# phlash/java-sdr

Hardware: NVIDIA B200
Metric: Msamples/s (complex IQ) through mix+FIR+FFT (higher is better)
Workload: dtype f32 (FFT/PSD) + f64 (tuner/decimator, reference order, bit-exact)

## Files before the change

include/jsdrcuda.h:

```cpp
#ifndef JSDRCUDA_H
#define JSDRCUDA_H

#include <stddef.h>
#include <stdint.h>

#ifdef __cplusplus
extern "C" {
#endif

#define JSDR_ABI_VERSION 2

typedef enum jsdr_status {
    JSDR_OK = 0,
    JSDR_EINVAL = -1,
    JSDR_ECUDA = -2,
    JSDR_ENOMEM = -3,
    JSDR_EUNSUPPORTED = -4,
    JSDR_ESTATE = -5,
    JSDR_EINTERNAL = -6
} jsdr_status;

enum { JSDR_MEM_HOST = 0, JSDR_MEM_DEVICE = 1 };

typedef struct jsdr_ctx jsdr_ctx;
// ... 82 lines not shown
                        int32_t *pixels, int mem);

int jsdr_fir_design(int f1, int f2, float rate, double w[21]);
int jsdr_fir_nco_table(int freq, float rate, int32_t *sig );
int jsdr_fir_create(jsdr_ctx *ctx, int nchan, int max_block_samples, jsdr_fir **out);
int jsdr_fir_destroy(jsdr_fir *f);
int jsdr_fir_set_weights(jsdr_fir *f, int chan, const double w[21]);
int jsdr_fir_filter_i32(jsdr_fir *f, const int32_t *in, int nsamples, int64_t chan_stride,
                        int32_t *out , int mem);
int jsdr_fir_complex_mod_i32(jsdr_ctx *ctx, const int32_t *a, const int32_t *b, int32_t *out,
                             int64_t npairs, int mem);

int jsdr_probe_table(int which, int32_t *out, int n);
int jsdr_probe_taps(double ds27[27], double dm65[65]);
int jsdr_probe_scout_thresholds(double inc, double *th1, double *th2);

int jsdr_pump_receive_s16(jsdr_fft *f, jsdr_bpsk *b, const int16_t *raw, int nblocks,
                          int ic, int qc, float *psd, int32_t *peak_bin, int mem);
int jsdr_pump_waterfall_s16(jsdr_fft *f, jsdr_bpsk *b, const int16_t *raw, int nblocks,
                            int ic, int qc, int width, uint32_t peak_rgb, int32_t *pixels,
                            float *peak, int32_t *peak_bin, int mem);

#ifdef __cplusplus
}
#endif
#endif
```

java-sdr_b200/csrc/bpsk.cu:

```cuda
#include <math.h>

#include <algorithm>
#include <cmath>
#include <stdlib.h>
#include <string.h>

#include <vector>

#include "fft_generic.cuh"
#include "handles.h"

namespace jsdr {
namespace bpsk {

constexpr double kTwoPi = 2.0 * 3.141592653589793;
constexpr double kInvTwoPi = 1.0 / kTwoPi;
constexpr int kTileOut = 128;
constexpr int kTileThreads = 128;
constexpr int kPrefetch = 21;
constexpr double kIdxScaleHi = 40.74366543152521;
constexpr double kIdxScaleLo = -9.306125250357089e-16;
constexpr int kDmTile = 128;

enum { FMT_F32 = 0, FMT_S16 = 1 };
// ... 163 lines not shown
            ph = p[k];
            const double ic = par[ch].inc;
            for (int w = 0; w < nfull; w++) {
                ckpt[(size_t)w * nchan + ch] = ph;
#pragma unroll 4
                for (int j = 0; j < 32; j++) ph = phase_step(ph, ic);
            }
        }
        if (S & 31) {
            const double ic = par[ch].inc;
            ckpt[(size_t)nfull * nchan + ch] = ph;
            for (int j = 0; j < (S & 31); j++) ph = phase_step(ph, ic);
        }
        phase_out[ch] = ph;
    }
}

__global__ void k_vco_scout(const double *__restrict__ state, double *__restrict__ state_out,
                            uint8_t *__restrict__ vco_ix, uint8_t *__restrict__ bit_roll, int NO, double vco_inc,
                            double bit_inc, double bit_time)
{
    if (threadIdx.x == 0) {
        double p = state[0];
        for (int m = 0; m < NO; m++) {
            p = phase_step(p, vco_inc);
            double q = __ddiv_rn(__dmul_rn(p, 256.0), kTwoPi);
            vco_ix[m] = (uint8_t)(__double2int_rz(q) & 255);
        }
        state_out[0] = p;
    } else if (threadIdx.x == 32) {
// ... 582 lines not shown
        return from_bits(lo);
    };
    th1 = last_false(wraps1);
    th2 = last_false(wraps2);
}

static ScoutChan scout_chan(double inc)
{
    ScoutChan c;
    c.inc = inc;
    c.th1 = c.th2 = c.pad = 0.0;
    if (inc > 0.0 && inc < 3.1) scout_thresholds(inc, c.th1, c.th2);
    return c;
}

int launch_scout(jsdr_bpsk *b, jsdr_bpsk::TunerPlan &P, int S)
{
    jsdr_ctx *ctx = b->ctx;
    ProfScope prof(ctx, JSDR_K_SCOUT, ctx->side);
    const int st = scout_threads(b), cpt = scout_cpt(b);
    static int scout_smem = 0;
    if (!scout_smem) scout_smem = env_int("JSDR_SCOUT_SMEM_KB", 1, 200, kScoutSmem / 1024) * 1024;
    static PerDeviceFlag attr_done;
    JSDR_TRY(attr_done.once(ctx->device, [&]() -> int {
        JSDR_CUDA(cudaFuncSetAttribute(k_tuner_scout<1>, cudaFuncAttributeMaxDynamicSharedMemorySize, scout_smem));
        JSDR_CUDA(cudaFuncSetAttribute(k_tuner_scout<2>, cudaFuncAttributeMaxDynamicSharedMemorySize, scout_smem));
        JSDR_CUDA(cudaFuncSetAttribute(k_tuner_scout<3>, cudaFuncAttributeMaxDynamicSharedMemorySize, scout_smem));
        JSDR_CUDA(cudaFuncSetAttribute(k_tuner_scout<4>, cudaFuncAttributeMaxDynamicSharedMemorySize, scout_smem));
        return JSDR_OK;
    }));
    const int per_cta = st * cpt;
    const int grid = (b->nchan + per_cta - 1) / per_cta;
    void (*kern)(const ScoutChan *, const double *, double *, double *, int, int) =
        cpt == 1 ? k_tuner_scout<1> : cpt == 2 ? k_tuner_scout<2> : cpt == 3 ? k_tuner_scout<3> : k_tuner_scout<4>;
// ... 112 lines not shown
    sp.in = mp.in;
    sp.chan_stride = mp.chan_stride;
    sp.S = S;
    sp.ic = mp.ic;
    sp.qc = mp.qc;
    sp.tu_dx56 = b->d_tu_dx56;
    sp.tu_inc = mp.tu_inc;
    sp.ckpt = mp.ckpt;
    sp.nchan = mp.nchan;
    sp.nchunks = (S + 31) / 32;
    sp.hist_in = mp.hist_in;
    sp.cossin = mp.cossin;
    sp.n0 = mp.n0;
    sp.NO = mp.NO;
    sp.ncw = (mp.nchan + 31) / 32;
    const int scout_ctas = (mp.nchan + scout_threads(b) - 1) / scout_threads(b);
    sp.grid = b->in_pump ? b->ctx->sm_count : std::max(b->ctx->sm_count - scout_ctas, b->ctx->sm_count / 2);
    sp.warps_per_cta = (FMT == FMT_S16) ? stream::kWarps : stream::kWarpsF32;
    const int resident = sp.grid * sp.warps_per_cta;
    static int segs_per_warp = 0;
    if (!segs_per_warp) segs_per_warp = env_int("JSDR_STREAM_SEGS", 1, 64, 10);
    int nseg = std::max(1, segs_per_warp * resident / sp.ncw);
    int R = (mp.NO + nseg - 1) / nseg;
    if (R < 64) R = 64;
    sp.R = R;
    sp.nseg = (mp.NO + R - 1) / R;
    sp.ds_out = mp.ds_out;
    sp.max_ds = mp.max_ds;
    sp.work_counter = reinterpret_cast<unsigned *>(b->d_nbits + b->nchan);
    for (int k = 0; k < stream::kMaxTaps; k++) {
        sp.taps[k] = (k < b->ntaps) ? b->h_taps[k] : 0.0;
        sp.tapsf[k] = (float)sp.taps[k];
// ... 82 lines not shown
        JSDR_CUDA(cudaMemsetAsync(b->d_nbits, 0, sizeof(int32_t) * b->nchan, ctx->aux));
        if (b->fec && b->stages >= 3 && b->d_bits) JSDR_TRY(jsdr_fec_after_bits(b));
        return JSDR_OK;
    }
    const int D = b->D;
    const int NO = (b->ds_cnt + S) / D;
    const int n0 = D - 1 - b->ds_cnt;
    const int nchan = b->nchan;

    jsdr_bpsk::TunerPlan &P = b->plan[b->plan_cur];
    const bool autotune = b->dofft != 0;
    if (autotune) JSDR_REQUIRE(S == b->max_block, JSDR_EINVAL, "auto-tune needs whole blocks of max_block_samples");
    JSDR_CUDA(cudaEventRecord(ctx->ev_fork, ctx->stream));
    JSDR_CUDA(cudaStreamWaitEvent(ctx->side, ctx->ev_fork, 0));
    JSDR_CUDA(cudaStreamWaitEvent(ctx->side2, ctx->ev_fork, 0));
    if (!autotune && !(P.valid && P.S == S)) JSDR_TRY(launch_scout(b, P, S));
    const int kb = b->bit_cur;
    if (b->stages >= 2 && NO > 0) {
        if (!(b->vco_ahead_valid && b->vco_ahead_NO == NO && b->vco_ahead_kb == kb)) JSDR_TRY(launch_vco_scout(b, NO, kb));
        b->vco_ahead_valid = false;
    }
    JSDR_CUDA(cudaEventRecord(ctx->ev_join, ctx->side));

    const void *d_in = in;
    if (mem == JSDR_MEM_HOST) {
        const size_t esz = (FMT == FMT_S16) ? 4 : 8;
        const size_t total = (chan_stride == 0) ? (size_t)S : (size_t)chan_stride * (nchan - 1) + S;
        if (b->in_cap < total * esz) {
            cudaFree(b->d_in);
            b->d_in = nullptr;
            b->in_cap = 0;
// ... 63 lines not shown
        kern<<<grid, kTileThreads, smem, ctx->stream>>>(mp);
        JSDR_TRY(launched(ctx, "k_mixdecim"));
    }
    if (b->ntaps > 1) {
        k_tuner_tail<FMT><<<nchan, 128, 0, ctx->stream>>>(mp);
        JSDR_TRY(launched(ctx, "k_tuner_tail"));
    }
    JSDR_CUDA(cudaEventRecord(P.consumed, ctx->stream));
    P.used = true;
    P.valid = false;
    b->d_tu_phase = P.phase_end;
    b->plan_cur ^= 1;
    {
        jsdr_bpsk::TunerPlan &Pn = b->plan[b->plan_cur];
        if (Pn.used) JSDR_CUDA(cudaStreamWaitEvent(ctx->side, Pn.consumed, 0));
        JSDR_TRY(launch_scout(b, Pn, S));
    }
    }
    b->ds_hist_cur ^= 1;
    b->ds_cnt = (b->ds_cnt + S) % D;
    b->cnt_raw += S;
    b->last_nds = NO;

    if (b->stages >= 2 && NO > 0) {
        JSDR_CUDA(cudaStreamWaitEvent(ctx->stream, b->ev_vco_ready, 0));
        b->vco_state_cur ^= 1;
        DmParams dp;
        dp.ds = b->d_ds_out;
        dp.max_ds = b->max_ds;
        dp.NO = NO;
        dp.vco_ix = b->d_vco_ix[kb];
// ... 96 lines not shown
            cudaGetLastError();                                      \
            return JSDR_ENOMEM;                                      \
        }                                                            \
        cudaMemsetAsync((ptr), 0, (bytes), ctx->stream);             \
    } while (0)
    ALLOC(b->d_taps, sizeof(double) * kMaxDsTaps);
    ALLOC(b->d_dmtaps, sizeof(double) * kDmTaps);
    ALLOC(b->d_cossin, sizeof(double) * 512);
    ALLOC(b->d_cossin2, sizeof(double2) * 257);
    ALLOC(b->d_tu_inc, sizeof(double) * nc);
    ALLOC(b->d_tu_par, sizeof(ScoutChan) * nc);
    ALLOC(b->d_tu_dx, sizeof(unsigned long long) * nc);
    ALLOC(b->d_tu_dx56, sizeof(unsigned long long) * nc);
    ALLOC(b->d_tu_phase0, sizeof(double) * nc);
    b->d_tu_phase = b->d_tu_phase0;
    for (int i = 0; i < 2; i++) {
        ALLOC(b->plan[i].ckpt, sizeof(double) * nc * b->max_words);
        ALLOC(b->plan[i].phase_end, sizeof(double) * nc);
        cudaEventCreateWithFlags(&b->plan[i].ready, cudaEventDisableTiming);
        cudaEventCreateWithFlags(&b->plan[i].consumed, cudaEventDisableTiming);
    }
    ALLOC(b->d_ds_hist[0], sizeof(double2) * kMaxDsTaps * nc);
    ALLOC(b->d_ds_hist[1], sizeof(double2) * kMaxDsTaps * nc);
    ALLOC(b->d_ds_out, sizeof(double2) * nc * b->max_ds);
    ALLOC(b->d_vco_state, sizeof(double) * 4);
    ALLOC(b->d_ts, sizeof(TimingState) * nc);
    ALLOC(b->d_nbits, sizeof(int32_t) * (nc + 1));
#undef ALLOC
    std::vector<double> cossin(512);
    for (int n = 0; n < 256; n++) {
// ... 16 lines not shown
        cs2[2 * n + 1] = cossin[256 + n];
    }
    cs2[512] = cs2[513] = 1.0;
    for (int i = 0; i < kMaxDsTaps; i++) b->h_taps[i] = taps[i];
    std::vector<TimingState> ts(nchan);
    memset(ts.data(), 0, sizeof(TimingState) * nc);
    for (int c = 0; c < nchan; c++) ts[c].dmEnergyOut = 1.0;
    int rc = upload(ctx, b->d_cossin, cossin.data(), sizeof(double) * 512);
    if (rc == JSDR_OK) rc = upload(ctx, b->d_taps, taps.data(), sizeof(double) * kMaxDsTaps);
    if (rc == JSDR_OK) rc = upload(ctx, b->d_dmtaps, dmt.data(), sizeof(double) * kDmTaps);
    if (rc == JSDR_OK) rc = upload(ctx, b->d_tu_inc, inc.data(), sizeof(double) * nc);
    if (rc == JSDR_OK) {
        std::vector<ScoutChan> par(nchan);
        for (int c = 0; c < nchan; c++) par[c] = scout_chan(inc[c]);
        rc = upload(ctx, b->d_tu_par, par.data(), sizeof(ScoutChan) * nc);
    }
    if (rc == JSDR_OK) rc = upload(ctx, b->d_tu_dx, dx.data(), sizeof(unsigned long long) * nc);
    if (rc == JSDR_OK) rc = upload(ctx, b->d_tu_dx56, dx56.data(), sizeof(unsigned long long) * nc);
    if (rc == JSDR_OK) rc = upload(ctx, b->d_cossin2, cs2.data(), sizeof(double) * 2 * 257);
    if (rc == JSDR_OK) rc = upload(ctx, b->d_ts, ts.data(), sizeof(TimingState) * nc);
    if (rc != JSDR_OK) {
        jsdr_bpsk_destroy(b);
        return rc;
    }
    *out = b;
    return JSDR_OK;
} JSDR_CATCH_ALL

extern "C" int jsdr_bpsk_destroy(jsdr_bpsk *b)
try {
    if (!b) return JSDR_OK;
    b->ctx->bind();
    cudaStreamSynchronize(b->ctx->side);
    cudaStreamSynchronize(b->ctx->side2);
    cudaStreamSynchronize(b->ctx->stream);
    cudaStreamSynchronize(b->ctx->aux);
    if (b->ds_read_pending) cudaStreamSynchronize(b->ctx->copy_out);
    if (b->ev_dm_ready) cudaEventDestroy(b->ev_dm_ready);
    if (b->ev_vco_ready) cudaEventDestroy(b->ev_vco_ready);
    if (b->ev_ds_ready) cudaEventDestroy(b->ev_ds_ready);
    if (b->ev_ds_read) cudaEventDestroy(b->ev_ds_read);
    for (int i = 0; i < 2; i++)
        if (b->ev_bits_done[i]) cudaEventDestroy(b->ev_bits_done[i]);
    void *ptrs[] = {b->d_taps, b->d_dmtaps, b->d_cossin, b->d_tu_inc, b->d_tu_par, b->d_tu_phase0, b->d_tu_dx, b->d_tu_dx56, b->d_cossin2, b->plan[0].ckpt, b->plan[0].phase_end, b->plan[1].ckpt, b->plan[1].phase_end,
                    b->d_ds_hist[0], b->d_ds_hist[1], b->d_ds_out, b->d_vco_state, b->d_vco_ix[0], b->d_vco_ix[1],
                    b->d_bit_roll[0], b->d_bit_roll[1], b->d_dm_hist[0], b->d_dm_hist[1], b->d_dm_buf[0], b->d_dm_buf[1], b->d_ts, b->d_bits,
                    b->d_bit_at, b->d_nbits, b->d_in, b->d_at_work[0], b->d_at_work[1], b->d_at_rev[0], b->d_at_rev[1], b->d_at_state};
    for (void *p : ptrs) cudaFree(p);
    jsdr_fec_destroy(b);
    for (int i = 0; i < 2; i++) {
        if (b->plan[i].ready) cudaEventDestroy(b->plan[i].ready);
        if (b->plan[i].consumed) cudaEventDestroy(b->plan[i].consumed);
    }
    delete b;
    return JSDR_OK;
} JSDR_CATCH_ALL

extern "C" int jsdr_bpsk_set_stages(jsdr_bpsk *b, int stages)
try {
// ... 49 lines not shown
try {
    JSDR_REQUIRE(b && chan >= 0 && chan < b->nchan, JSDR_EINVAL, "bad channel");
    JSDR_REQUIRE(std::isfinite(hz), JSDR_EINVAL, "tuning must be a finite frequency (the reference's comes from an int config key or the dialog, :175-195)");
    JSDR_TRY(b->ctx->bind());
    JSDR_CUDA(cudaStreamSynchronize(b->ctx->side));
    JSDR_CUDA(cudaStreamSynchronize(b->ctx->side2));
    b->plan[0].valid = b->plan[1].valid = false;
    b->h_tuning[chan] = hz;
    double inc = 2.0 * M_PI * hz / (double)b->rate;
    unsigned long long dx = index_step_fixed(inc);
    JSDR_TRY(upload(b->ctx, b->d_tu_dx + chan, &dx, sizeof(dx)));
    unsigned long long dx56 = index_step_fixed56(inc);
    JSDR_TRY(upload(b->ctx, b->d_tu_dx56 + chan, &dx56, sizeof(dx56)));
    const ScoutChan sc = scout_chan(inc);
    JSDR_TRY(upload(b->ctx, b->d_tu_par + chan, &sc, sizeof(sc)));
    return upload(b->ctx, b->d_tu_inc + chan, &inc, sizeof(double));
} JSDR_CATCH_ALL

extern "C" int jsdr_bpsk_set_ds_filter(jsdr_bpsk *b, const double *taps, int ntaps)
try {
    JSDR_REQUIRE(b && taps && ntaps >= 1 && ntaps <= kMaxDsTaps, JSDR_EINVAL, "1..128 taps");
    JSDR_TRY(b->ctx->bind());
    std::vector<double> t(kMaxDsTaps, 0.0);
    for (int i = 0; i < ntaps; i++) t[i] = taps[i];
    JSDR_TRY(upload(b->ctx, b->d_taps, t.data(), sizeof(double) * kMaxDsTaps));
    for (int i = 0; i < kMaxDsTaps; i++) b->h_taps[i] = t[i];
    b->ntaps = ntaps;
    return bpsk_reset_ds(b);
} JSDR_CATCH_ALL

// ... 268 lines not shown
extern "C" int jsdr_probe_taps(double *ds27, double *dm65)
try {
    JSDR_REQUIRE(ds27 && dm65, JSDR_EINVAL, "null argument");
    for (int i = 0; i < 27; i++) ds27[i] = (double)jsdr::bpsk::kDsFilterF[i];
    for (int i = 0; i < 65; i++) dm65[i] = (double)jsdr::bpsk::kDmFilterF[i];
    return JSDR_OK;
} JSDR_CATCH_ALL

extern "C" int jsdr_probe_scout_thresholds(double inc, double *th1, double *th2)
try {
    JSDR_REQUIRE(th1 && th2, JSDR_EINVAL, "null argument");
    JSDR_REQUIRE(inc > 0.0 && inc < 3.1, JSDR_EINVAL, "the pair form covers 0 < inc < 3.1");
    scout_thresholds(inc, *th1, *th2);
    return JSDR_OK;
} JSDR_CATCH_ALL
```

java-sdr_b200/csrc/handles.h:

```cpp
#pragma once

#include <stddef.h>
#include <stdint.h>

#include <vector>

#include "common.cuh"

struct jsdr_fft {
    jsdr_ctx *ctx = nullptr;
    int n = 0, rate = 0, max_batch = 0;
    void *launch = nullptr;
    float2 *d_tw = nullptr;
    float2 *d_work[2] = {nullptr, nullptr};
    unsigned long long *d_best = nullptr;
    int fs_n1 = 0;
    int split = 0;
    float2 *d_tw2 = nullptr;
    unsigned *d_cnt = nullptr;
    void *d_in = nullptr;
    float *d_out = nullptr;
    int32_t *d_peak = nullptr;
    size_t in_cap = 0, out_cap = 0;
    int32_t *d_pix = nullptr;
// ... 5 lines not shown

struct TimingState {
    double dmEnergy[8];
    double dmEnergyOut;
    double lastI, lastQ;
    int bitPos, peakPos, newPeak, pad;
    long long cntBit;
};

struct AutoTuneState {
    double avePeakPower, aveCentreBin;
    int centreBin, pad;
};

struct ScoutChan;
constexpr int kMaxDsTaps = 128;
constexpr int kDmTaps = 65;

}
}

struct jsdr_fec_state;
int jsdr_launch_waterfall(jsdr_ctx *ctx, const float *d_psd, int n, int rows, int width, uint32_t peak_rgb,
                          int32_t *d_pix, cudaStream_t st);

struct jsdr_bpsk {
    jsdr_ctx *ctx = nullptr;
    jsdr_fec_state *fec = nullptr;
    int rate = 0, D = 0, nchan = 0, max_block = 0, stages = 3;
    int ntaps = 27;
    int max_ds = 0, max_words = 0, max_bits = 0;
    std::vector<double> h_tuning;

    double *d_taps = nullptr;
    double *d_dmtaps = nullptr;
    double *d_cossin = nullptr;
    double2 *d_cossin2 = nullptr;

    double *d_tu_inc = nullptr;
    jsdr::bpsk::ScoutChan *d_tu_par = nullptr;
    unsigned long long *d_tu_dx = nullptr;
    unsigned long long *d_tu_dx56 = nullptr;
    int precision = 0;
    int kernel_mode = 0;
    int in_pump = 0;
    double *d_tu_phase0 = nullptr;
    const double *d_tu_phase = nullptr;
    struct TunerPlan {
        double *ckpt = nullptr;
        double *phase_end = nullptr;
        int S = 0;
        bool valid = false;
        bool used = false;
        cudaEvent_t ready = nullptr, consumed = nullptr;
    } plan[2];
    int plan_cur = 0;
    double h_taps[128] = {0};
    double2 *d_ds_hist[2] = {nullptr, nullptr};
    int ds_hist_cur = 0;
    int ds_cnt = 0;
// ... 79 lines not shown
```

java-sdr_b200/jsdrcuda/__init__.py:

```python
from __future__ import annotations

import ctypes as C
import os
import subprocess

import numpy as np

_PKG = os.path.dirname(os.path.abspath(__file__))
_ROOT = os.path.dirname(_PKG)
_SO = os.path.join(_ROOT, "libjsdrcuda.so")
HEADER = os.path.join(os.path.dirname(_ROOT), "include", "jsdrcuda.h")

MEM_HOST, MEM_DEVICE = 0, 1
PREC_F64, PREC_F32 = 0, 1
KERNEL_AUTO, KERNEL_TILE, KERNEL_STREAM, KERNEL_PRING = 0, 1, 2, 3
INT_MIN = -2147483648


class JsdrError(RuntimeError):
    def __init__(self, code: int, msg: str):
        super().__init__(f"jsdrcuda error {code}: {msg}")
        self.code = code


# ... 26 lines not shown
    "jsdr_memcpy_h2d": [_vp, _vp, _vp, C.c_size_t],
    "jsdr_memcpy_d2h": [_vp, _vp, _vp, C.c_size_t],
    "jsdr_memset_dev": [_vp, _vp, _i, C.c_size_t],
    "jsdr_timer_start": [_vp],
    "jsdr_timer_stop_ms": [_vp, C.POINTER(_f)],
    "jsdr_fft_supported": [_i],
    "jsdr_fft_create": [_vp, _i, _i, _i, _pp],
    "jsdr_fft_destroy": [_vp],
    "jsdr_fft_receive_f32": [_vp, _vp, _i, _vp, _vp, _i],
    "jsdr_fft_receive_s16": [_vp, _vp, _i, _i, _i, _vp, _vp, _i],
    "jsdr_fft_forward_f32": [_vp, _vp, _i, _vp, _i],
    "jsdr_bpsk_create": [_vp, _i, _i, _vp, _i, _pp],
    "jsdr_bpsk_destroy": [_vp],
    "jsdr_bpsk_set_stages": [_vp, _i],
    "jsdr_bpsk_set_tuning": [_vp, _i, _d],
    "jsdr_bpsk_set_autotune": [_vp, _i, _i],
    "jsdr_bpsk_read_centre": [_vp, _vp],
    "jsdr_bpsk_enable_fec": [_vp, _vp, _i],
    "jsdr_bpsk_read_frames": [_vp, _vp, _vp, _vp, _vp, _vp, _i],
    "jsdr_bpsk_read_fec_counters": [_vp, _vp, _vp],
    "jsdr_bpsk_set_precision": [_vp, _i],
    "jsdr_bpsk_set_kernel": [_vp, _i],
    "jsdr_bpsk_set_ds_filter": [_vp, _vp, _i],
    "jsdr_bpsk_receive_f32": [_vp, _vp, _i, _i64, _i],
    "jsdr_bpsk_receive_s16": [_vp, _vp, _i, _i64, _i, _i, _i],
    "jsdr_bpsk_last_counts": [_vp, C.POINTER(C.c_int32)],
    "jsdr_bpsk_read_ds": [_vp, _vp, _i],
    "jsdr_bpsk_read_ds_async": [_vp, _vp, _i],
    "jsdr_bpsk_read_dm": [_vp, _vp, _i],
    "jsdr_bpsk_read_bits": [_vp, _vp, _vp, _vp, _i, _i],
# ... 8 lines not shown
    "jsdr_demod_set_mode": [_vp, _i, _i],
    "jsdr_demod_receive_audio_f32": [_vp, _vp, _i, _i64, _vp, _vp, _i],
    "jsdr_waterfall_rows": [_vp, _vp, _i, _i, _i, C.c_uint32, _vp, _i],
    "jsdr_fir_design": [_i, _i, _f, _vp],
    "jsdr_fir_nco_table": [_i, _f, _vp],
    "jsdr_fir_create": [_vp, _i, _i, _pp],
    "jsdr_fir_destroy": [_vp],
    "jsdr_fir_set_weights": [_vp, _i, _vp],
    "jsdr_fir_filter_i32": [_vp, _vp, _i, _i64, _vp, _i],
    "jsdr_fir_complex_mod_i32": [_vp, _vp, _vp, _vp, _i64, _i],
    "jsdr_pump_receive_s16": [_vp, _vp, _vp, _i, _i, _i, _vp, _vp, _i],
    "jsdr_pump_waterfall_s16": [_vp, _vp, _vp, _i, _i, _i, _i, C.c_uint32, _vp, _vp, _vp, _i],
    "jsdr_probe_table": [_i, _vp, _i],
    "jsdr_probe_taps": [_vp, _vp],
    "jsdr_probe_scout_thresholds": [_d, C.POINTER(_d), C.POINTER(_d)],
}
EXPORTS = sorted(list(_SIGS) + ["jsdr_last_error"])


def lib() -> C.CDLL:
    global _lib
    if _lib is None:
        if not os.path.exists(_SO):
            raise ImportError(f"{_SO} is missing: run `python -c 'import __graft_entry__ as g; g.build()'` "
                              "(there is no CPU fallback)")
        _lib = C.CDLL(os.environ.get("JSDR_LIB") or _SO)
        for name, args in _SIGS.items():
            fn = getattr(_lib, name, None)
            if fn is None:
                if os.environ.get("JSDR_LIB"):
# ... 231 lines not shown
        h = C.c_void_p()
        _ck(lib().jsdr_bpsk_create(ctx.h, adsc.rate, self.nchan, _ptr(self.tuning), self.max_block, C.byref(h)))
        self.h = h
        self.stages = stages
        _ck(lib().jsdr_bpsk_set_stages(h, stages))

    def close(self):
        if self.h:
            lib().jsdr_bpsk_destroy(self.h)
            self.h = None

    def set_tuning(self, chan: int, hz: float):
        _ck(lib().jsdr_bpsk_set_tuning(self.h, chan, hz))
        self.tuning[chan] = hz

    def set_autotune(self, dofft: bool, upper: bool = False):
        self.dofft = bool(dofft)
        _ck(lib().jsdr_bpsk_set_autotune(self.h, int(dofft), int(upper)))

    def centre_bins(self) -> np.ndarray:
        out = np.zeros(self.nchan, dtype=np.int32)
        _ck(lib().jsdr_bpsk_read_centre(self.h, _ptr(out)))
        return out

    def enable_fec(self, mettab: np.ndarray, max_frames: int = 64):
        t = np.ascontiguousarray(mettab, dtype=np.int16).reshape(2, 256)
        self._max_frames = max_frames
        _ck(lib().jsdr_bpsk_enable_fec(self.h, _ptr(t), max_frames))

    def read_frames(self):
# ... 214 lines not shown


def probe_table(name: str) -> np.ndarray:
    which, n = _TABLE_SIZES[name]
    out = np.empty(n, dtype=np.int32)
    _ck(lib().jsdr_probe_table(which, _ptr(out), n))
    return out


def probe_scout_thresholds(inc: float):
    a, b = _d(), _d()
    _ck(lib().jsdr_probe_scout_thresholds(inc, C.byref(a), C.byref(b)))
    return a.value, b.value


def probe_taps():
    ds, dm = np.empty(27), np.empty(65)
    _ck(lib().jsdr_probe_taps(_ptr(ds), _ptr(dm)))
    return ds, dm
```

Measured before the change: 269,200.

## Parallelize serial tuner phase scout via precomputed wrap-jump tables

Replaces the serial per-channel phase recurrence scout with a two-stage scheme. Host-built per-channel piecewise tables map the fixed-point phase after a wrap to the phase and step count J wraps later. A jump kernel uses them to find restart states across the block, and a fill kernel replays the segments in parallel to write checkpoints bit-exactly. The goal is to shorten the long serial dependency chain on the side stream and to free SMs for the main streaming kernel. The cost is host table construction on tuning changes, extra device memory, and a fallback to the serial path when table building fails.

```diff
diff --git a/include/jsdrcuda.h b/include/jsdrcuda.h
--- a/include/jsdrcuda.h
+++ b/include/jsdrcuda.h
@@ -120,6 +120,10 @@
 int jsdr_probe_table(int which, int32_t *out, int n);
 int jsdr_probe_taps(double ds27[27], double dm65[65]);
 int jsdr_probe_scout_thresholds(double inc, double *th1, double *th2);
+int jsdr_bpsk_replay_tuner(jsdr_bpsk *b, const double *phase_in, int nsamples, int serial, double *ckpt,
+                           double *phase_out);
+int jsdr_probe_tuner_jump(const double *inc, const double *phase_in, int nchan, int S, double *ckpt,
+                          double *phase_out, int32_t *J, int32_t *pieces);
 
 int jsdr_pump_receive_s16(jsdr_fft *f, jsdr_bpsk *b, const int16_t *raw, int nblocks,
                           int ic, int qc, float *psd, int32_t *peak_bin, int mem);
diff --git a/java-sdr_b200/csrc/bpsk.cu b/java-sdr_b200/csrc/bpsk.cu
--- a/java-sdr_b200/csrc/bpsk.cu
+++ b/java-sdr_b200/csrc/bpsk.cu
@@ -5,6 +5,7 @@
 #include <stdlib.h>
 #include <string.h>
 
+#include <thread>
 #include <vector>
 
 #include "fft_generic.cuh"
@@ -201,6 +202,155 @@
         }
         phase_out[ch] = ph;
     }
+}
+
+struct JumpChan {
+    long long bucket;
+    int nb;
+    int shift;
+};
+struct __align__(16) JumpPiece {
+    unsigned long long lo;
+    long long dk;
+};
+constexpr int kJumpMaxK = 1023;
+constexpr int kJumpMinK = 128;
+constexpr int kJumpThreads = 128;
+
+__host__ __device__ __forceinline__ double add_rn(double a, double b)
+{
+#ifdef __CUDA_ARCH__
+    return __dadd_rn(a, b);
+#else
+    volatile double s = a + b;
+    return s;
+#endif
+}
+
+__host__ __device__ __forceinline__ unsigned ld_keep(const unsigned *p)
+{
+#ifdef __CUDA_ARCH__
+    unsigned v;
+    unsigned long long pol;
+    asm("createpolicy.fractional.L2::evict_last.b64 %0, 1.0;" : "=l"(pol));
+    asm volatile("ld.global.nc.L2::cache_hint.u32 %0, [%1], %2;" : "=r"(v) : "l"(p), "l"(pol));
+    return v;
+#else
+    return *p;
+#endif
+}
+__host__ __device__ __forceinline__ JumpPiece ld_keep(const JumpPiece *p)
+{
+#ifdef __CUDA_ARCH__
+    JumpPiece v;
+    unsigned long long pol, lo, dk;
+    asm("createpolicy.fractional.L2::evict_last.b64 %0, 1.0;" : "=l"(pol));
+    asm volatile("ld.global.nc.L2::cache_hint.v2.u64 {%0, %1}, [%2], %3;" : "=l"(lo), "=l"(dk) : "l"(p), "l"(pol));
+    v.lo = lo;
+    v.dk = (long long)dk;
+    return v;
+#else
+    return *p;
+#endif
+}
+
+__host__ __device__ __forceinline__ int jump_states(double p, double inc, int S, const JumpChan &jc,
+                                                    const JumpPiece *__restrict__ piece,
+                                                    const unsigned *__restrict__ bucket, int cap, int *rec_n,
+                                                    double *rec_p, size_t stride)
+{
+    rec_n[0] = 0;
+    rec_p[0] = p;
+    if (jc.shift < 0 || !(p >= 0.0 && p <= kTwoPi)) return 1;
+    int n = 0;
+    for (;;) {
+        if (n == S) return 1;
+        const double a = add_rn(p, inc);
+        n++;
+        if (a > kTwoPi) {
+            p = add_rn(a, -kTwoPi);
+            break;
+        }
+        p = a;
+    }
+    unsigned long long R = (unsigned long long)(p * 1125899906842624.0);
+    int cnt = 1;
+    while (n < S && cnt < cap) {
+        rec_n[cnt * stride] = n;
+        rec_p[cnt * stride] = (double)R * (1.0 / 1125899906842624.0);
+        cnt++;
+        unsigned i = ld_keep(bucket + jc.bucket + (long long)(R & 3) * jc.nb + (long long)((R - 1) >> jc.shift));
+        JumpPiece pc = ld_keep(piece + i), nx = ld_keep(piece + i + 1);
+        while (nx.lo <= R) {
+            pc = nx;
+            nx = ld_keep(piece + ++i + 1);
+        }
+        const long long dk = pc.dk;
+        R += (unsigned long long)(dk >> 10);
+        n += (int)(dk & 1023);
+    }
+    return cnt;
+}
+
+__global__ void __launch_bounds__(kJumpThreads)
+k_tuner_jump(const ScoutChan *__restrict__ par, const JumpChan *__restrict__ jch, const JumpPiece *__restrict__ piece,
+             const unsigned *__restrict__ bucket, const double *__restrict__ phase_in, int *__restrict__ rec_n,
+             double *__restrict__ rec_p, int *__restrict__ nrec, int cap, int nchan, int S)
+{
+    const int ch = blockIdx.x * blockDim.x + threadIdx.x;
+    if (ch >= nchan) return;
+    nrec[ch] = jump_states(phase_in[ch], par[ch].inc, S, jch[ch], piece, bucket, cap, rec_n + ch, rec_p + ch, nchan);
+}
+
+__device__ __forceinline__ void fill_one(const ScoutChan *__restrict__ par, const int *__restrict__ rec_n,
+                                         const double *__restrict__ rec_p, const int *__restrict__ nrec,
+                                         double *__restrict__ phase_out, double *__restrict__ ckpt, int nchan, int S,
+                                         int k, int ch)
+{
+    if (ch >= nchan) return;
+    const int nr = nrec[ch];
+    if (k >= nr) return;
+    const size_t o = (size_t)k * nchan + ch;
+    int n = rec_n[o];
+    double p = rec_p[o];
+    const int e = (k + 1 < nr) ? rec_n[o + nchan] : S;
+    const ScoutChan c = par[ch];
+    const bool pair = c.inc > 0.0 && c.inc < 3.1 && p >= 0.0 && p <= kTwoPi;
+    auto steps = [&](int m) {
+        if (pair)
+            for (; m >= 2; m -= 2) p = phase_step2(p, c.inc, c.th1, c.th2);
+        for (; m > 0; m--) p = phase_step(p, c.inc);
+    };
+    if (n & 31) {
+        const int m = min(e, (n + 31) & ~31) - n;
+        steps(m);
+        n += m;
+    }
+    for (; n + 32 <= e; n += 32) {
+        ckpt[(size_t)(n >> 5) * nchan + ch] = p;
+        if (pair) {
+#pragma unroll
+            for (int j = 0; j < 16; j++) p = phase_step2(p, c.inc, c.th1, c.th2);
+        } else {
+#pragma unroll 4
+            for (int j = 0; j < 32; j++) p = phase_step(p, c.inc);
+        }
+    }
+    if (n < e) {
+        ckpt[(size_t)(n >> 5) * nchan + ch] = p;
+        steps(e - n);
+    }
+    if (k + 1 == nr) phase_out[ch] = p;
+}
+
+__global__ void __launch_bounds__(kJumpThreads)
+k_tuner_fill(const ScoutChan *__restrict__ par, const int *__restrict__ rec_n, const double *__restrict__ rec_p,
+             const int *__restrict__ nrec, double *__restrict__ phase_out, double *__restrict__ ckpt, int nchan, int S,
+             int nitems)
+{
+    const int ngrp = (nchan + kJumpThreads - 1) / kJumpThreads;
+    for (int it = blockIdx.x; it < nitems; it += gridDim.x)
+        fill_one(par, rec_n, rec_p, nrec, phase_out, ckpt, nchan, S, it / ngrp, (it % ngrp) * kJumpThreads + threadIdx.x);
 }
 
 __global__ void k_vco_scout(const double *__restrict__ state, double *__restrict__ state_out,
@@ -813,10 +963,225 @@
     return c;
 }
 
-int launch_scout(jsdr_bpsk *b, jsdr_bpsk::TunerPlan &P, int S)
+static double jump_target() { static int v = -1; if (v < 0) v = env_int("JSDR_JUMP_L", 64, 1000, 256); return v; }
+namespace jump {
+struct Piece {
+    unsigned long long lo, hi;
+    long long d;
+    int k;
+};
+struct Fail {};
+struct Sig {
+    long long d = 0;
+    int k = 0;
+    std::vector<signed char> bin;
+};
+constexpr size_t kMaxPieces = 4096;
+
+static Sig cycle(double inc, unsigned long long R)
+{
+    Sig s;
+    volatile double q = std::ldexp((double)R, -50);
+    for (int k = 1; k <= kJumpMaxK; k++) {
+        volatile double a = q + inc;
+        q = a;
+        s.bin.push_back((signed char)std::ilogb(a));
+        if (a > kTwoPi) {
+            volatile double w = a - kTwoPi;
+            const double r2 = std::ldexp((double)w, 50);
+            if (r2 != std::floor(r2) || r2 < 1.0) throw Fail();
+            s.k = k;
+            s.d = (long long)r2 - (long long)R;
+            return s;
+        }
+    }
+    throw Fail();
+}
+
+static void split(double inc, unsigned long long lo, unsigned long long hi, const Sig &a, const Sig &b,
+                  std::vector<Piece> &out)
+{
+    if (a.bin == b.bin) {
+        if (a.d != b.d) throw Fail();
+        out.push_back({lo, hi, a.d, a.k});
+    } else if (hi - lo == 4) {
+        out.push_back({lo, lo, a.d, a.k});
+        out.push_back({hi, hi, b.d, b.k});
+    } else {
+        const unsigned long long mid = lo + 4 * ((hi - lo) / 8);
+        split(inc, lo, mid, a, cycle(inc, mid), out);
+        split(inc, mid + 4, hi, cycle(inc, mid + 4), b, out);
+    }
+    if (out.size() > kMaxPieces) throw Fail();
+}
+
+static void merge(std::vector<Piece> &v)
+{
+    std::vector<Piece> m;
+    for (const Piece &p : v) {
+        if (!m.empty() && m.back().d == p.d && m.back().k == p.k) m.back().hi = p.hi;
+        else m.push_back(p);
+    }
+    v.swap(m);
+}
+}
+
+static bool build_jump_table(double inc, JumpTable &t)
+{
+    using namespace jump;
+    if (!(inc > 0.0 && inc < 3.1) || 2.0 * M_PI / inc > 0.5 * kJumpMaxK) return false;
+    try {
+        const unsigned long long rmax = (unsigned long long)std::floor(std::ldexp(inc, 50)) + 2;
+        std::vector<Piece> M[4];
+        for (int r = 0; r < 4; r++) {
+            const unsigned long long lo = r ? (unsigned long long)r : 4, hi = rmax - ((rmax - r) & 3);
+            split(inc, lo, hi, cycle(inc, lo), cycle(inc, hi), M[r]);
+            merge(M[r]);
+        }
+        int kmin1 = 1 << 30;
+        for (auto &v : M)
+            for (auto &p : v) kmin1 = std::min(kmin1, p.k);
+        const int J = std::max((int)std::ceil(jump_target() * inc / (2.0 * M_PI)), (kJumpMinK + kmin1 - 1) / kmin1);
+        std::vector<Piece> MJ[4] = {M[0], M[1], M[2], M[3]};
+        for (int j = 1; j < J; j++) {
+            for (int r = 0; r < 4; r++) {
+                std::vector<Piece> nx;
+                for (const Piece &p : MJ[r]) {
+                    const unsigned long long a = p.lo + p.d, b = p.hi + p.d;
+                    const std::vector<Piece> &m = M[a & 3];
+                    size_t i = std::lower_bound(m.begin(), m.end(), a, [](const Piece &x, unsigned long long v) { return x.hi < v; }) - m.begin();
+                    unsigned long long cur = a;
+                    for (; i < m.size() && m[i].lo <= b; i++) {
+                        if (m[i].lo > cur) throw Fail();
+                        const unsigned long long e = std::min(b, m[i].hi);
+                        nx.push_back({cur - p.d, e - p.d, p.d + m[i].d, p.k + m[i].k});
+                        cur = e + 4;
+                    }
+                    if (cur <= b) throw Fail();
+                }
+                merge(nx);
+                if (nx.size() > kMaxPieces) throw Fail();
+                MJ[r].swap(nx);
+            }
+        }
+        int kmin = 1 << 30, kmax = 0;
+        size_t npmax = 0;
+        for (auto &v : MJ) {
+            npmax = std::max(npmax, v.size());
+            for (auto &p : v) kmin = std::min(kmin, p.k), kmax = std::max(kmax, p.k);
+        }
+        if (kmax > kJumpMaxK || kmin < kJumpMinK) return false;
+        int s = 0;
+        while (((rmax - 1) >> s) + 1 > 2 * npmax) s++;
+        const int nb = (int)(((rmax - 1) >> s) + 1);
+        t = JumpTable();
+        t.J = J, t.kmin = kmin, t.kmax = kmax, t.shift = s, t.nb = nb;
+        t.buckets.resize((size_t)4 * nb);
+        for (int r = 0; r < 4; r++) {
+            const unsigned base = (unsigned)t.lo.size();
+            size_t i = 0;
+            for (int b = 0; b < nb; b++) {
+                const unsigned long long start = 1 + ((unsigned long long)b << s);
+                while (i + 1 < MJ[r].size() && MJ[r][i + 1].lo <= start) i++;
+                t.buckets[(size_t)r * nb + b] = base + (unsigned)i;
+            }
+            for (const Piece &p : MJ[r]) {
+                t.lo.push_back(p.lo);
+                t.dk.push_back(p.d * 1024 + p.k);
+            }
+            t.lo.push_back(~0ull);
+            t.dk.push_back(0);
+        }
+        return true;
+    } catch (Fail &) {
+        t = JumpTable();
+        return false;
+    }
+}
+
+static void build_jump_tables(const double *inc, std::vector<JumpTable> &out, int nchan)
+{
+    const int nt = std::max(1, std::min<int>((int)std::thread::hardware_concurrency(), (nchan + 63) / 64));
+    std::vector<std::thread> th;
+    for (int w = 0; w < nt; w++)
+        th.emplace_back([&, w]() {
+            for (int c = w; c < nchan; c += nt) build_jump_table(inc[c], out[c]);
+        });
+    for (auto &x : th) x.join();
+}
+
+static int upload_jump_tables(jsdr_bpsk *b)
+{
+    std::vector<JumpChan> ch(b->nchan);
+    std::vector<JumpPiece> pc;
+    std::vector<unsigned> bk;
+    int kmin = 0;
+    for (int c = 0; c < b->nchan; c++) {
+        const JumpTable &t = b->h_jump[c];
+        ch[c].bucket = (long long)bk.size();
+        ch[c].nb = t.nb;
+        ch[c].shift = t.lo.empty() ? -1 : t.shift;
+        if (t.lo.empty()) continue;
+        const unsigned base = (unsigned)pc.size();
+        for (size_t i = 0; i < t.lo.size(); i++) pc.push_back({t.lo[i], t.dk[i]});
+        for (unsigned x : t.buckets) bk.push_back(base + x);
+        kmin = kmin ? std::min(kmin, t.kmin) : t.kmin;
+    }
+    cudaFree(b->d_jump_piece);
+    cudaFree(b->d_jump_bucket);
+    b->d_jump_piece = nullptr;
+    b->d_jump_bucket = nullptr;
+    b->jump_kmin = 0;
+    if (!pc.empty()) {
+        JSDR_CUDA(cudaMalloc((void **)&b->d_jump_piece, sizeof(JumpPiece) * pc.size()));
+        JSDR_CUDA(cudaMalloc((void **)&b->d_jump_bucket, sizeof(unsigned) * bk.size()));
+        JSDR_TRY(upload(b->ctx, b->d_jump_piece, pc.data(), sizeof(JumpPiece) * pc.size()));
+        JSDR_TRY(upload(b->ctx, b->d_jump_bucket, bk.data(), sizeof(unsigned) * bk.size()));
+    }
+    JSDR_TRY(upload(b->ctx, b->d_jump_chan, ch.data(), sizeof(JumpChan) * ch.size()));
+    b->jump_kmin = kmin;
+    return JSDR_OK;
+}
+
+static bool scout_serial()
+{
+    static int v = -1;
+    if (v < 0) {
+        const char *e = getenv("JSDR_SCOUT");
+        v = (e && !strcmp(e, "serial")) ? 1 : 0;
+    }
+    return v == 1;
+}
+
+static bool scout_by_jumps(const jsdr_bpsk *b)
+{
+    const char *e = getenv("JSDR_SCOUT");
+    if (e && !strcmp(e, "jump")) return true;
+    return !scout_serial() && !b->in_pump && b->stages == 1;
+}
+
+int launch_scout(jsdr_bpsk *b, jsdr_bpsk::TunerPlan &P, int S, bool serial)
 {
     jsdr_ctx *ctx = b->ctx;
     ProfScope prof(ctx, JSDR_K_SCOUT, ctx->side);
+    if (!serial) {
+        const int nblk = (b->nchan + kJumpThreads - 1) / kJumpThreads;
+        k_tuner_jump<<<nblk, kJumpThreads, 0, ctx->side>>>(b->d_tu_par, b->d_jump_chan, b->d_jump_piece, b->d_jump_bucket,
+                                                           b->d_tu_phase, b->d_rec_n, b->d_rec_p, b->d_nrec, b->rec_cap,
+                                                           b->nchan, S);
+        JSDR_TRY(launched(ctx, "k_tuner_jump"));
+        const int nrec = b->jump_kmin ? std::min(b->rec_cap, S / b->jump_kmin + 3) : 1;
+        const int per_sm = env_int("JSDR_FILL_CTAS", 0, 16, 0);
+        const int nitems = nrec * nblk;
+        const int fgrid = per_sm ? std::min(nitems, per_sm * ctx->sm_count) : nitems;
+        k_tuner_fill<<<fgrid, kJumpThreads, 0, ctx->side>>>(b->d_tu_par, b->d_rec_n, b->d_rec_p, b->d_nrec,
+                                                             P.phase_end, P.ckpt, b->nchan, S, nitems);
+        JSDR_TRY(launched(ctx, "k_tuner_fill"));
+        JSDR_CUDA(cudaEventRecord(P.ready, ctx->side));
+        P.S = S;
+        P.valid = true;
+        return JSDR_OK;
+    }
     const int st = scout_threads(b), cpt = scout_cpt(b);
     static int scout_smem = 0;
     if (!scout_smem) scout_smem = env_int("JSDR_SCOUT_SMEM_KB", 1, 200, kScoutSmem / 1024) * 1024;
@@ -959,8 +1324,9 @@
     sp.n0 = mp.n0;
     sp.NO = mp.NO;
     sp.ncw = (mp.nchan + 31) / 32;
-    const int scout_ctas = (mp.nchan + scout_threads(b) - 1) / scout_threads(b);
-    sp.grid = b->in_pump ? b->ctx->sm_count : std::max(b->ctx->sm_count - scout_ctas, b->ctx->sm_count / 2);
+    const int scout_ctas = !scout_by_jumps(b) ? (mp.nchan + scout_threads(b) - 1) / scout_threads(b)
+                                              : std::min(16, (mp.nchan + kJumpThreads - 1) / kJumpThreads);
+    sp.grid = b->in_pump ? b->ctx->sm_count - env_int("JSDR_PUMP_RESERVE", 0, 64, 0) : std::max(b->ctx->sm_count - scout_ctas, b->ctx->sm_count / 2);
     sp.warps_per_cta = (FMT == FMT_S16) ? stream::kWarps : stream::kWarpsF32;
     const int resident = sp.grid * sp.warps_per_cta;
     static int segs_per_warp = 0;
@@ -1073,7 +1439,7 @@
     JSDR_CUDA(cudaEventRecord(ctx->ev_fork, ctx->stream));
     JSDR_CUDA(cudaStreamWaitEvent(ctx->side, ctx->ev_fork, 0));
     JSDR_CUDA(cudaStreamWaitEvent(ctx->side2, ctx->ev_fork, 0));
-    if (!autotune && !(P.valid && P.S == S)) JSDR_TRY(launch_scout(b, P, S));
+    if (!autotune && !(P.valid && P.S == S)) JSDR_TRY(launch_scout(b, P, S, !scout_by_jumps(b)));
     const int kb = b->bit_cur;
     if (b->stages >= 2 && NO > 0) {
         if (!(b->vco_ahead_valid && b->vco_ahead_NO == NO && b->vco_ahead_kb == kb)) JSDR_TRY(launch_vco_scout(b, NO, kb));
@@ -1167,7 +1533,7 @@
     {
         jsdr_bpsk::TunerPlan &Pn = b->plan[b->plan_cur];
         if (Pn.used) JSDR_CUDA(cudaStreamWaitEvent(ctx->side, Pn.consumed, 0));
-        JSDR_TRY(launch_scout(b, Pn, S));
+        JSDR_TRY(launch_scout(b, Pn, S, !scout_by_jumps(b)));
     }
     }
     b->ds_hist_cur ^= 1;
@@ -1294,6 +1660,11 @@
     ALLOC(b->d_tu_dx56, sizeof(unsigned long long) * nc);
     ALLOC(b->d_tu_phase0, sizeof(double) * nc);
     b->d_tu_phase = b->d_tu_phase0;
+    ALLOC(b->d_jump_chan, sizeof(JumpChan) * nc);
+    b->rec_cap = b->max_block / kJumpMinK + 3;
+    ALLOC(b->d_rec_n, sizeof(int) * nc * b->rec_cap);
+    ALLOC(b->d_rec_p, sizeof(double) * nc * b->rec_cap);
+    ALLOC(b->d_nrec, sizeof(int) * nc);
     for (int i = 0; i < 2; i++) {
         ALLOC(b->plan[i].ckpt, sizeof(double) * nc * b->max_words);
         ALLOC(b->plan[i].phase_end, sizeof(double) * nc);
@@ -1340,6 +1711,11 @@
         std::vector<ScoutChan> par(nchan);
         for (int c = 0; c < nchan; c++) par[c] = scout_chan(inc[c]);
         rc = upload(ctx, b->d_tu_par, par.data(), sizeof(ScoutChan) * nc);
+    }
+    if (rc == JSDR_OK) {
+        b->h_jump.assign(nchan, JumpTable());
+        build_jump_tables(inc.data(), b->h_jump, nchan);
+        rc = upload_jump_tables(b);
     }
     if (rc == JSDR_OK) rc = upload(ctx, b->d_tu_dx, dx.data(), sizeof(unsigned long long) * nc);
     if (rc == JSDR_OK) rc = upload(ctx, b->d_tu_dx56, dx56.data(), sizeof(unsigned long long) * nc);
@@ -1369,6 +1745,7 @@
     for (int i = 0; i < 2; i++)
         if (b->ev_bits_done[i]) cudaEventDestroy(b->ev_bits_done[i]);
     void *ptrs[] = {b->d_taps, b->d_dmtaps, b->d_cossin, b->d_tu_inc, b->d_tu_par, b->d_tu_phase0, b->d_tu_dx, b->d_tu_dx56, b->d_cossin2, b->plan[0].ckpt, b->plan[0].phase_end, b->plan[1].ckpt, b->plan[1].phase_end,
+                    b->d_jump_chan, b->d_jump_piece, b->d_jump_bucket, b->d_rec_n, b->d_rec_p, b->d_nrec,
                     b->d_ds_hist[0], b->d_ds_hist[1], b->d_ds_out, b->d_vco_state, b->d_vco_ix[0], b->d_vco_ix[1],
                     b->d_bit_roll[0], b->d_bit_roll[1], b->d_dm_hist[0], b->d_dm_hist[1], b->d_dm_buf[0], b->d_dm_buf[1], b->d_ts, b->d_bits,
                     b->d_bit_at, b->d_nbits, b->d_in, b->d_at_work[0], b->d_at_work[1], b->d_at_rev[0], b->d_at_rev[1], b->d_at_state};
@@ -1448,6 +1825,8 @@
     JSDR_TRY(upload(b->ctx, b->d_tu_dx56 + chan, &dx56, sizeof(dx56)));
     const ScoutChan sc = scout_chan(inc);
     JSDR_TRY(upload(b->ctx, b->d_tu_par + chan, &sc, sizeof(sc)));
+    build_jump_table(inc, b->h_jump[chan]);
+    JSDR_TRY(upload_jump_tables(b));
     return upload(b->ctx, b->d_tu_inc + chan, &inc, sizeof(double));
 } JSDR_CATCH_ALL
 
@@ -1746,3 +2125,82 @@
     scout_thresholds(inc, *th1, *th2);
     return JSDR_OK;
 } JSDR_CATCH_ALL
+
+extern "C" int jsdr_probe_tuner_jump(const double *inc, const double *phase_in, int nchan, int S, double *ckpt,
+                                     double *phase_out, int32_t *J, int32_t *pieces)
+try {
+    JSDR_REQUIRE(inc && phase_in && ckpt && phase_out && nchan > 0 && S >= 0, JSDR_EINVAL, "bad argument");
+    std::vector<JumpTable> tab(nchan);
+    build_jump_tables(inc, tab, nchan);
+    const int nt = std::max(1, std::min<int>((int)std::thread::hardware_concurrency(), nchan));
+    std::vector<std::thread> th;
+    for (int w = 0; w < nt; w++)
+        th.emplace_back([&, w]() {
+            const int cap = S / kJumpMinK + 3;
+            std::vector<int> rn(cap);
+            std::vector<double> rp(cap);
+            for (int c = w; c < nchan; c += nt) {
+                const JumpTable &t = tab[c];
+                std::vector<JumpPiece> pc;
+                for (size_t i = 0; i < t.lo.size(); i++) pc.push_back({t.lo[i], t.dk[i]});
+                const JumpChan jc = {0, t.nb, t.lo.empty() ? -1 : t.shift};
+                const int nr = jump_states(phase_in[c], inc[c], S, jc, pc.data(), t.buckets.data(), cap, rn.data(), rp.data(), 1);
+                for (int k = 0; k < nr; k++) {
+                    double p = rp[k];
+                    const int e = (k + 1 < nr) ? rn[k + 1] : S;
+                    for (int n = rn[k]; n < e; n++) {
+                        if (!(n & 31)) ckpt[(size_t)(n >> 5) * nchan + c] = p;
+                        volatile double a = p + inc[c];
+                        p = a;
+                        if (p > kTwoPi) {
+                            volatile double q = p - kTwoPi;
+                            p = q;
+                        }
+                    }
+                    if (k + 1 == nr) phase_out[c] = p;
+                }
+                if (J) J[c] = t.J;
+                if (pieces) pieces[c] = t.lo.empty() ? 0 : (int)t.lo.size() - 4;
+            }
+        });
+    for (auto &x : th) x.join();
+    return JSDR_OK;
+} JSDR_CATCH_ALL
+
+extern "C" int jsdr_bpsk_replay_tuner(jsdr_bpsk *b, const double *phase_in, int S, int serial, double *ckpt,
+                                      double *phase_out)
+try {
+    JSDR_REQUIRE(b && phase_in && ckpt && phase_out, JSDR_EINVAL, "null argument");
+    JSDR_REQUIRE(S >= 0 && S <= b->max_block, JSDR_EINVAL, "nsamples exceeds max_block_samples");
+    jsdr_ctx *ctx = b->ctx;
+    JSDR_TRY(ctx->bind());
+    JSDR_CUDA(cudaStreamSynchronize(ctx->side));
+    const size_t nc = (size_t)b->nchan, nw = (size_t)(S + 31) / 32;
+    jsdr_bpsk::TunerPlan P;
+    double *d_in = nullptr;
+    int rc = JSDR_OK;
+    if (cudaMalloc((void **)&d_in, sizeof(double) * nc) != cudaSuccess ||
+        cudaMalloc((void **)&P.ckpt, sizeof(double) * nc * std::max<size_t>(nw, 1)) != cudaSuccess ||
+        cudaMalloc((void **)&P.phase_end, sizeof(double) * nc) != cudaSuccess ||
+        cudaEventCreateWithFlags(&P.ready, cudaEventDisableTiming) != cudaSuccess) {
+        cudaGetLastError();
+        set_error("jsdr_bpsk_replay_tuner: out of device memory");
+        rc = JSDR_ENOMEM;
+    }
+    const double *committed = b->d_tu_phase;
+    if (rc == JSDR_OK) rc = upload(ctx, d_in, phase_in, sizeof(double) * nc);
+    if (rc == JSDR_OK) {
+        b->d_tu_phase = d_in;
+        rc = launch_scout(b, P, S, serial != 0);
+        b->d_tu_phase = committed;
+    }
+    if (rc == JSDR_OK && cudaStreamSynchronize(ctx->side) != cudaSuccess) rc = JSDR_ECUDA;
+    if (rc == JSDR_OK && nw) rc = cudaMemcpy(ckpt, P.ckpt, sizeof(double) * nc * nw, cudaMemcpyDeviceToHost) == cudaSuccess ? JSDR_OK : JSDR_ECUDA;
+    if (rc == JSDR_OK) rc = cudaMemcpy(phase_out, P.phase_end, sizeof(double) * nc, cudaMemcpyDeviceToHost) == cudaSuccess ? JSDR_OK : JSDR_ECUDA;
+    if (rc == JSDR_ECUDA) set_error("jsdr_bpsk_replay_tuner: %s", cudaGetErrorString(cudaGetLastError()));
+    cudaFree(d_in);
+    cudaFree(P.ckpt);
+    cudaFree(P.phase_end);
+    if (P.ready) cudaEventDestroy(P.ready);
+    return rc;
+} JSDR_CATCH_ALL
diff --git a/java-sdr_b200/csrc/handles.h b/java-sdr_b200/csrc/handles.h
--- a/java-sdr_b200/csrc/handles.h
+++ b/java-sdr_b200/csrc/handles.h
@@ -43,6 +43,14 @@
 };
 
 struct ScoutChan;
+struct JumpChan;
+struct JumpPiece;
+struct JumpTable {
+    int J = 0, kmin = 0, kmax = 0, shift = -1, nb = 0;
+    std::vector<unsigned long long> lo;
+    std::vector<long long> dk;
+    std::vector<unsigned> buckets;
+};
 constexpr int kMaxDsTaps = 128;
 constexpr int kDmTaps = 65;
 
@@ -73,6 +81,15 @@
     int precision = 0;
     int kernel_mode = 0;
     int in_pump = 0;
+    std::vector<jsdr::bpsk::JumpTable> h_jump;
+    jsdr::bpsk::JumpChan *d_jump_chan = nullptr;
+    jsdr::bpsk::JumpPiece *d_jump_piece = nullptr;
+    unsigned *d_jump_bucket = nullptr;
+    int jump_kmin = 0;
+    int rec_cap = 0;
+    int *d_rec_n = nullptr;
+    double *d_rec_p = nullptr;
+    int *d_nrec = nullptr;
     double *d_tu_phase0 = nullptr;
     const double *d_tu_phase = nullptr;
     struct TunerPlan {
diff --git a/java-sdr_b200/jsdrcuda/__init__.py b/java-sdr_b200/jsdrcuda/__init__.py
--- a/java-sdr_b200/jsdrcuda/__init__.py
+++ b/java-sdr_b200/jsdrcuda/__init__.py
@@ -64,6 +64,7 @@
     "jsdr_bpsk_destroy": [_vp],
     "jsdr_bpsk_set_stages": [_vp, _i],
     "jsdr_bpsk_set_tuning": [_vp, _i, _d],
+    "jsdr_bpsk_replay_tuner": [_vp, _vp, _i, _i, _vp, _vp],
     "jsdr_bpsk_set_autotune": [_vp, _i, _i],
     "jsdr_bpsk_read_centre": [_vp, _vp],
     "jsdr_bpsk_enable_fec": [_vp, _vp, _i],
@@ -102,6 +103,7 @@
     "jsdr_probe_table": [_i, _vp, _i],
     "jsdr_probe_taps": [_vp, _vp],
     "jsdr_probe_scout_thresholds": [_d, C.POINTER(_d), C.POINTER(_d)],
+    "jsdr_probe_tuner_jump": [_vp, _vp, _i, _i, _vp, _vp, _vp, _vp],
 }
 EXPORTS = sorted(list(_SIGS) + ["jsdr_last_error"])
 
@@ -363,6 +365,14 @@
         _ck(lib().jsdr_bpsk_set_tuning(self.h, chan, hz))
         self.tuning[chan] = hz
 
+    def replay_tuner(self, phase_in, nsamples: int, serial: bool = False):
+        phase_in = np.ascontiguousarray(phase_in, dtype=np.float64)
+        assert phase_in.size == self.nchan
+        ckpt = np.empty(((nsamples + 31) // 32, self.nchan))
+        out = np.empty(self.nchan)
+        _ck(lib().jsdr_bpsk_replay_tuner(self.h, _ptr(phase_in), nsamples, int(serial), _ptr(ckpt), _ptr(out)))
+        return ckpt, out
+
     def set_autotune(self, dofft: bool, upper: bool = False):
         self.dofft = bool(dofft)
         _ck(lib().jsdr_bpsk_set_autotune(self.h, int(dofft), int(upper)))
@@ -607,6 +617,19 @@
     return a.value, b.value
 
 
+def probe_tuner_jump(inc, phase_in, S: int):
+    inc = np.ascontiguousarray(inc, dtype=np.float64)
+    phase_in = np.ascontiguousarray(phase_in, dtype=np.float64)
+    n = inc.size
+    assert phase_in.size == n
+    ckpt = np.empty(((S + 31) // 32, n))
+    out = np.empty(n)
+    J = np.empty(n, dtype=np.int32)
+    pieces = np.empty(n, dtype=np.int32)
+    _ck(lib().jsdr_probe_tuner_jump(_ptr(inc), _ptr(phase_in), n, S, _ptr(ckpt), _ptr(out), _ptr(J), _ptr(pieces)))
+    return ckpt, out, J, pieces
+
+
 def probe_taps():
     ds, dm = np.empty(27), np.empty(65)
     _ck(lib().jsdr_probe_taps(_ptr(ds), _ptr(dm)))
```

New measurement: 269,200, median of 6. No clear change (-0.0%).
